# kaushik87599/Melo-GAN

Hardware: AMD Instinct MI355X
Metric: piano-roll samples/sec (G+D step), batch=64 128x256 roll (higher is better)
Workload: dtype f32; 1 GPU; cfg2: 128x256 piano-roll, batch=64 per GPU, full G+D+emotion-D step (1 critic update incl. gradient penalty + 1 generator update); global_batch=64, T=256, C=128, parallelism=dp1, graph=True

## Files before the change

melo-gan_amd/csrc/wgrad_mfma.hip:

```cpp
#include "common.h"
#include <stdlib.h>
#include <type_traits>

namespace {

struct WgradP {
    const float* s[2];
    const float* l[2];
    int nb[2];
    float* part;
    float* out;
    float* bias_out;
    int Ts, Tl, A, Bc;
    int tt_log2, n_ttiles;
    int bps;
    int n_bgroups;
    int nbg0;
    long slab;
    long wslab;
    int bias_from;
    int nseg_bias;
    int vec_ok;
    int lin;
    int gx, gy, gz;
};

constexpr int RT = 64;
constexpr int BA = 32, BB = 32;

typedef unsigned u32x4 __attribute__((ext_vector_type(4)));

#ifdef MG_STAMPS
__device__ long long* mg_wstamp_buf = nullptr;
#define MG_STAMP(k)                                                                                        \
    do {                                                                                                   \
        if (threadIdx.x == 0 && mg_wstamp_buf)                                                             \
            mg_wstamp_buf[((long)(blockIdx.z * gridDim.y + blockIdx.y) * gridDim.x + blockIdx.x) * 8 + (k)] = \
                wall_clock64();                                                                            \
    } while (0)
#else
#define MG_STAMP(k)
#endif

template <int S, int K>
__device__ __forceinline__ void wgrad_body(const WgradP& p, const int bx, const int by, const int bz) {
    constexpr int PAD = (K - 1) / 2;
    constexpr int RMAX = (RT - 1) * S + K;
    constexpr int NS4 = RT * (BA / 4) / 256;
    constexpr int NL4 = (RMAX * (BB / 4) + 255) / 256 + 1;
    extern __shared__ __attribute__((aligned(16))) float smem[];
    const int tid = threadIdx.x, lane = tid & 63, wave = tid >> 6;
    MG_STAMP(0);
    const int TT = 1 << p.tt_log2, TB = RT >> p.tt_log2;
    const int R = (TT - 1) * S + K;
    const int lrows = TB * R;
    float* Ss = smem;
    float* Ls = smem + RT * BA;
    const int a0 = bx * BA, b0 = by * BB;
    const int split = bz;

    f32x16 acc[K];
#pragma unroll
    for (int k = 0; k < K; ++k)
#pragma unroll
        for (int r = 0; r < 16; ++r) acc[k][r] = 0.f;

    const int h = lane >> 5;
    const int g_begin = split * p.bps;
    const int g_end = min(g_begin + p.bps, p.n_bgroups);
    const int n_chunks = (g_end - g_begin) * p.n_ttiles;

    auto compute = [&]() {
#ifdef MG_EXP_NOMMA
        return;
#endif
#pragma unroll
        for (int r2 = 0; r2 < RT / 8; ++r2) {
            const int r = wave * (RT / 4) + 2 * r2 + h;
            const int seg = r >> p.tt_log2, tl = r & (TT - 1);
            const float av = Ss[r * BA + (lane & 31)];
            const float* lrow = Ls + (seg * R + tl * S) * BB + (lane & 31);
#pragma unroll
            for (int k = 0; k < K; ++k)
                acc[k] = __builtin_amdgcn_mfma_f32_32x32x2f32(av, lrow[k * BB], acc[k], 0, 0, 0);
        }
    };

    const bool fast = ((p.A & 3) == 0) && ((p.Bc & 3) == 0) && p.vec_ok && (lrows * (BB / 4) <= 256 * NL4);
    if (fast) {
        float4 sr[NS4], lr[NL4];
        auto load_chunk = [&](int c) {
            const int g = g_begin + c / p.n_ttiles, tt = c - (c / p.n_ttiles) * p.n_ttiles;
            const int seg_id = g < p.nbg0 ? 0 : 1;
            const int bg = seg_id ? g - p.nbg0 : g;
            const int nb = p.nb[seg_id];
            const int bb0 = bg * TB, t0 = tt * TT, tl0 = t0 * S - PAD;
            const __amdgpu_buffer_rsrc_t srs = __builtin_amdgcn_make_buffer_rsrc(
                const_cast<float*>(seg_id ? p.s[1] : p.s[0]), 0, (int)((long)nb * p.Ts * p.A * 4), 0x00020000);
            const __amdgpu_buffer_rsrc_t lrs = __builtin_amdgcn_make_buffer_rsrc(
                const_cast<float*>(seg_id ? p.l[1] : p.l[0]), 0, (int)((long)nb * p.Tl * p.Bc * 4), 0x00020000);
#pragma unroll
            for (int j = 0; j < NS4; ++j) {
                const int idx = tid + 256 * j;
                const int r = idx / (BA / 4), q = idx - r * (BA / 4);
                const int seg = r >> p.tt_log2, tl = r & (TT - 1);
                const int b = bb0 + seg, t = t0 + tl, a = a0 + 4 * q;
                unsigned off = 0x80000000u;
                if (b < nb && t < p.Ts && a < p.A) off = (unsigned)((((long)b * p.Ts + t) * p.A + a) * 4);
                const u32x4 v = __builtin_amdgcn_raw_buffer_load_b128(srs, off, 0, 0);
                sr[j] = make_float4(__uint_as_float(v[0]), __uint_as_float(v[1]), __uint_as_float(v[2]), __uint_as_float(v[3]));
            }
#pragma unroll
            for (int j = 0; j < NL4; ++j) {
                const int idx = tid + 256 * j;
                const int row = idx / (BB / 4), q = idx - row * (BB / 4);
                const int seg = row / R, rr = row - seg * R;
                const int b = bb0 + seg, t = tl0 + rr, cc = b0 + 4 * q;
                unsigned off = 0x80000000u;
                if (row < lrows && b < nb && t >= 0 && t < p.Tl && cc < p.Bc)
                    off = (unsigned)((((long)b * p.Tl + t) * p.Bc + cc) * 4);
                const u32x4 v = __builtin_amdgcn_raw_buffer_load_b128(lrs, off, 0, 0);
                lr[j] = make_float4(__uint_as_float(v[0]), __uint_as_float(v[1]), __uint_as_float(v[2]), __uint_as_float(v[3]));
            }
        };
        auto store_chunk = [&]() {
#pragma unroll
            for (int j = 0; j < NS4; ++j) *reinterpret_cast<float4*>(Ss + 4 * (tid + 256 * j)) = sr[j];
#pragma unroll
            for (int j = 0; j < NL4; ++j) {
                const int idx = tid + 256 * j;
                if (idx < lrows * (BB / 4)) *reinterpret_cast<float4*>(Ls + 4 * idx) = lr[j];
            }
        };
        if (n_chunks > 0) {
            load_chunk(0);
            store_chunk();
            __syncthreads();
            for (int c = 0; c < n_chunks; ++c) {
                const bool more = c + 1 < n_chunks;
#ifndef MG_EXP_NOLOADS
                if (more) load_chunk(c + 1);
#endif
                compute();
                __syncthreads();
                if (more) {
                    store_chunk();
                    __syncthreads();
                }
            }
        }
    } else {
        for (int g = g_begin; g < g_end; ++g) {
            const int seg_id = g < p.nbg0 ? 0 : 1;
            const int bg = seg_id ? g - p.nbg0 : g;
            const float* Sp = p.s[seg_id];
            const float* Lp = p.l[seg_id];
            const int nb = p.nb[seg_id];
            const int bb0 = bg * TB;
            for (int tt = 0; tt < p.n_ttiles; ++tt) {
                const int t0 = tt * TT;
                const int tl0 = t0 * S - PAD;
                __syncthreads();
                for (int idx = tid; idx < RT * BA; idx += 256) {
                    const int r = idx / BA, al = idx - r * BA;
                    const int seg = r >> p.tt_log2, tl = r & (TT - 1);
                    const int b = bb0 + seg, t = t0 + tl, a = a0 + al;
                    float v = 0.f;
                    if (b < nb && t < p.Ts && a < p.A) v = Sp[((long)b * p.Ts + t) * p.A + a];
                    Ss[r * BA + al] = v;
                }
                for (int idx = tid; idx < TB * R * BB; idx += 256) {
                    const int row = idx / BB, cl = idx - row * BB;
                    const int seg = row / R, rr = row - seg * R;
                    const int b = bb0 + seg, t = tl0 + rr, c = b0 + cl;
                    float v = 0.f;
                    if (b < nb && t >= 0 && t < p.Tl && c < p.Bc) v = Lp[((long)b * p.Tl + t) * p.Bc + c];
                    Ls[row * BB + cl] = v;
                }
                __syncthreads();
                compute();
            }
        }
    }

#ifdef MG_EXP_NOEPI
    if (acc[0][0] != 12345.f) return;
#endif
    MG_STAMP(2);
    float* red = smem;
    float* out = p.part ? p.part + (long)split * p.slab : p.out;
    constexpr int KP = K > 3 ? 3 : K;
    const int nb_cols = min(32, p.Bc - b0);
#pragma unroll
    for (int k0 = 0; k0 < K; k0 += KP) {
        const int kn = (K - k0) < KP ? (K - k0) : KP;
        __syncthreads();
#pragma unroll
        for (int k = k0; k < k0 + kn; ++k)
#pragma unroll
            for (int r = 0; r < 16; ++r)
                red[((wave * KP + (k - k0)) * 32 + (r & 3) + 8 * (r >> 2) + 4 * h) * 33 + (lane & 31)] = acc[k][r];
        __syncthreads();
#pragma unroll 4
        for (int idx = tid; idx < 32 * kn * 32; idx += 256) {
            const int ar = idx / (kn * 32), j = idx - ar * (kn * 32);
            const int bc = j / kn, kk = j - bc * kn;
            const int a = a0 + ar;
            const int o = (kk * 32 + ar) * 33 + bc;
            const float v = (red[o] + red[o + KP * 32 * 33]) + (red[o + 2 * KP * 32 * 33] + red[o + 3 * KP * 32 * 33]);
            if (a < p.A && bc < nb_cols) out[((long)a * p.Bc + b0 + bc) * K + k0 + kk] = v;
        }
    }
    MG_STAMP(3);
}

constexpr int W16_SP = 48;
template <int S> struct W16LP { static constexpr int value = S == 2 ? 40 : 48; };

template <int S, int K>
__device__ __forceinline__ bool wgrad16_applies(const WgradP& p) {
    constexpr int RMAX = (RT - 1) * S + K;
    constexpr int NL4 = (RMAX * (BB / 4) + 255) / 256 + 1;
    const int TT = 1 << p.tt_log2, TB = RT >> p.tt_log2, R = (TT - 1) * S + K;
    return ((p.A & 3) == 0) && ((p.Bc & 3) == 0) && p.vec_ok && (TB * R * (BB / 4) <= 256 * NL4) && p.tt_log2 >= 4;
}

template <int S, int K>
__device__ __forceinline__ void wgrad16_body(const WgradP& p, const int bx, const int by, const int bz) {
    constexpr int PAD = (K - 1) / 2;
    constexpr int RMAX = (RT - 1) * S + K;
    constexpr int NS4 = RT * (BA / 4) / 256;
    constexpr int NL4 = (RMAX * (BB / 4) + 255) / 256 + 1;
    constexpr int SP = W16_SP, LP = W16LP<S>::value;
    extern __shared__ __attribute__((aligned(16))) float smem[];
    const int tid = threadIdx.x, lane = tid & 63, wave = tid >> 6;
    const int li = lane & 15, kq = lane >> 4, wa = wave & 1, wb = wave >> 1;
    const int TT = 1 << p.tt_log2, TB = RT >> p.tt_log2;
    const int R = (TT - 1) * S + K;
    const int lrows = TB * R;
    const int a0 = bx * BA, b0 = by * BB;
    const int g_begin = bz * p.bps, g_end = min(g_begin + p.bps, p.n_bgroups);
    const int n_chunks = (g_end - g_begin) * p.n_ttiles;
    float* out = p.part ? p.part + (long)bz * p.slab : p.out;
    MG_STAMP(0);

    f32x4 acc[K];
#pragma unroll
    for (int k = 0; k < K; ++k) acc[k] = f32x4{0.f, 0.f, 0.f, 0.f};

    if (n_chunks > 0) {
        const int buf_floats = RT * SP + lrows * LP;
        const int sink = 2 * buf_floats + 4 * tid;
        constexpr unsigned DEAD = 0xC0000000u;
        int s_lds[NS4];
        unsigned s_base[NS4];
#pragma unroll
        for (int j = 0; j < NS4; ++j) {
            const int idx = tid + 256 * j, r = idx / (BA / 4), q = idx - r * (BA / 4);
            const int seg = r >> p.tt_log2, tl = r & (TT - 1);
            s_lds[j] = r * SP + 4 * q;
            s_base[j] = (unsigned)((((long)seg * p.Ts + tl) * p.A + a0 + 4 * q) * 4);
            if (a0 + 4 * q >= p.A || (TB > 1 && tl >= p.Ts)) s_base[j] = DEAD;
        }
        int l_lds[NL4], l_ldd[NL4];
        unsigned l_base[NL4];
#pragma unroll
        for (int j = 0; j < NL4; ++j) {
            const int idx = tid + 256 * j, row = idx / (BB / 4), q = idx - row * (BB / 4);
            const int seg = (TB == 1) ? 0 : row / R, rr = row - seg * R;
            const bool live = row < lrows;
            l_lds[j] = live ? RT * SP + row * LP + 4 * q : sink;
            l_ldd[j] = live ? buf_floats : 0;
            l_base[j] = (unsigned)(int)((((long)seg * p.Tl + rr - PAD) * p.Bc + b0 + 4 * q) * 4);
            if (!live || b0 + 4 * q >= p.Bc || (TB > 1 && (rr < PAD || rr - PAD >= p.Tl))) l_base[j] = DEAD;
        }
        f32x4 sr[NS4], lr[NL4];
        __amdgpu_buffer_rsrc_t srs, lrs;
        unsigned s_add = 0, l_add = 0;
        int nc = 0, ng = g_begin, ntt = 0;
        auto chunk_desc = [&]() {
            const int seg_id = ng < p.nbg0 ? 0 : 1;
            const int bg = seg_id ? ng - p.nbg0 : ng;
            const int bb0 = bg * TB;
            const int nbv = min(TB, p.nb[seg_id] - bb0);
            srs = __builtin_amdgcn_make_buffer_rsrc(const_cast<float*>((seg_id ? p.s[1] : p.s[0]) + (long)bb0 * p.Ts * p.A), 0,
                                                    nbv * p.Ts * p.A * 4, 0x00020000);
            lrs = __builtin_amdgcn_make_buffer_rsrc(const_cast<float*>((seg_id ? p.l[1] : p.l[0]) + (long)bb0 * p.Tl * p.Bc), 0,
                                                    nbv * p.Tl * p.Bc * 4, 0x00020000);
            const int t0 = ntt << p.tt_log2;
            s_add = (unsigned)(t0 * p.A * 4);
            l_add = (unsigned)(t0 * S * p.Bc * 4);
        };
        auto chunk_next = [&]() {
            if (nc + 1 < n_chunks) {
                ++nc;
                if (++ntt == p.n_ttiles) { ntt = 0; ++ng; }
            }
            chunk_desc();
        };
        auto bload = [&](const __amdgpu_buffer_rsrc_t& rsrc, unsigned off) {
            const u32x4 v = __builtin_amdgcn_raw_buffer_load_b128(rsrc, off, 0, 0);
            return f32x4{__uint_as_float(v[0]), __uint_as_float(v[1]), __uint_as_float(v[2]), __uint_as_float(v[3])};
        };
        auto lds4 = [&](int off) { return reinterpret_cast<f32x4*>(__builtin_assume_aligned(smem + off, 16)); };
        auto store_s = [&](int j, int buf) { *lds4(s_lds[j] + (buf ? buf_floats : 0)) = sr[j]; };
        auto store_l = [&](int j, int buf) { *lds4(l_lds[j] + (buf ? l_ldd[j] : 0)) = lr[j]; };

        const int abase = kq * SP + 16 * wa + li;
        const int lbase = RT * SP + kq * S * LP + 16 * wb + li;
        constexpr int NG = RT / 4;
        constexpr int NOPS = 2 * (NS4 + NL4);
        typedef float f32x8 __attribute__((ext_vector_type(8)));
        f32x8 fr[2];
        auto block_off = [&](int g) { return (((4 * g) >> p.tt_log2) * R + ((4 * g) & (TT - 1)) * S) * LP; };
        auto read_a = [&](int boff, int g, f32x8& v) { v[7] = smem[boff + abase + 4 * g * SP]; };
        auto read_b = [&](int boff, int g, int k, f32x8& v) { v[k] = smem[boff + lbase + block_off(g) + k * LP]; };
        auto chunk = [&](auto parity, int c) {
            constexpr int P = decltype(parity)::value;
            const int cur = P ? buf_floats : 0, oth = buf_floats - cur;
            chunk_next();
#pragma unroll
            for (int m = 0; m < NG * K; ++m) {
                const int g = m / K, k = m % K;
                acc[k] = __builtin_amdgcn_mfma_f32_16x16x4f32(fr[g & 1][7], fr[g & 1][k], acc[k], 0, 0, 0);
                const int gn = g + 1 < NG ? g + 1 : 0, bo = g + 1 < NG ? cur : oth;
                if (g + 1 == NG && k == 0) __syncthreads();
                if (k == 0) read_a(bo, gn, fr[(g + 1) & 1]);
                read_b(bo, gn, k, fr[(g + 1) & 1]);
                if (g + 1 < NG && k == K - 1) {
#pragma unroll
                    for (int o = 0; o < NOPS; ++o) {
                        if (o * (NG - 1) / NOPS != g) continue;
                        const int j = o / 2;
                        if (j < NS4) {
                            if (o % 2 == 0) store_s(j, 1 - P);
                            else sr[j] = bload(srs, s_base[j] + s_add);
                        } else {
                            if (o % 2 == 0) store_l(j - NS4, 1 - P);
                            else lr[j - NS4] = bload(lrs, l_base[j - NS4] + l_add);
                        }
                    }
                }
                __builtin_amdgcn_sched_barrier(0);
            }
        };
        auto load_all = [&]() {
#pragma unroll
            for (int j = 0; j < NS4; ++j) sr[j] = bload(srs, s_base[j] + s_add);
#pragma unroll
            for (int j = 0; j < NL4; ++j) lr[j] = bload(lrs, l_base[j] + l_add);
        };
        chunk_desc();
        load_all();
#pragma unroll
        for (int j = 0; j < NS4; ++j) store_s(j, 0);
#pragma unroll
        for (int j = 0; j < NL4; ++j) store_l(j, 0);
        if (n_chunks > 1) {
            chunk_next();
            load_all();
        }
        __syncthreads();
        read_a(0, 0, fr[0]);
#pragma unroll
        for (int k = 0; k < K; ++k) read_b(0, 0, k, fr[0]);
        MG_STAMP(1);
        for (int c = 0;;) {
            chunk(std::integral_constant<int, 0>{}, c);
            if (++c >= n_chunks) break;
            chunk(std::integral_constant<int, 1>{}, c);
            if (++c >= n_chunks) break;
        }
    }
    MG_STAMP(2);

    __syncthreads();
    constexpr int PE = K * 32 + 1;
    float* red = smem;
#pragma unroll
    for (int k = 0; k < K; ++k)
#pragma unroll
        for (int r = 0; r < 4; ++r) red[(16 * wa + 4 * kq + r) * PE + (16 * wb + li) * K + k] = acc[k][r];
    __syncthreads();
    const int nb_valid = min(32, p.Bc - b0) * K;
#pragma unroll 4
    for (int idx = tid; idx < 32 * K * 32; idx += 256) {
        const int ar = idx / (K * 32), j = idx - ar * (K * 32);
        if (a0 + ar < p.A && j < nb_valid) out[((long)(a0 + ar) * p.Bc + b0) * K + j] = red[ar * PE + j];
    }
    MG_STAMP(3);
}

constexpr int LIN_BB = 128;
__device__ __forceinline__ bool wgrad_lin_applies(const WgradP& p) {
    return p.lin != 0;
}
__device__ __forceinline__ void wgrad_lin_body(const WgradP& p, const int bx, const int by, const int bz) {
    extern __shared__ __attribute__((aligned(16))) float smem[];
    constexpr int SPL = 36, LPL = 132;
    float* Ss = smem;
    float* Ls = smem + RT * SPL;
    const int tid = threadIdx.x, lane = tid & 63, wave = tid >> 6, h = lane >> 5, c = lane & 31;
    const int a0 = bx * BA, b0 = by * LIN_BB;
    const int TB = RT;
    const int g_begin = bz * p.bps, g_end = min(g_begin + p.bps, p.n_bgroups);
    f32x16 acc;
#pragma unroll
    for (int i = 0; i < 16; ++i) acc[i] = 0.f;
    for (int g = g_begin; g < g_end; ++g) {
        const int seg_id = g < p.nbg0 ? 0 : 1;
        const int bb0 = (seg_id ? g - p.nbg0 : g) * TB;
        const int nb = p.nb[seg_id];
        const float* Sp = p.s[seg_id] + (long)bb0 * p.A;
        const float* Lp = p.l[seg_id] + (long)bb0 * p.Bc;
        const int rows = min(TB, nb - bb0);
        __syncthreads();
#pragma unroll
        for (int j = 0; j < 2; ++j) {
            const int idx = tid + 256 * j, r = idx >> 3, q = idx & 7;
            const bool ok = r < rows && a0 + 4 * q < p.A;
            const f32x4 v = *reinterpret_cast<const f32x4*>(Sp + (long)(ok ? r : 0) * p.A + (ok ? a0 + 4 * q : 0));
            *reinterpret_cast<f32x4*>(Ss + r * SPL + 4 * q) = ok ? v : f32x4{0.f, 0.f, 0.f, 0.f};
        }
#pragma unroll
        for (int j = 0; j < 8; ++j) {
            const int idx = tid + 256 * j, r = idx >> 5, q = idx & 31;
            const bool ok = r < rows && b0 + 4 * q < p.Bc;
            const f32x4 v = *reinterpret_cast<const f32x4*>(Lp + (long)(ok ? r : 0) * p.Bc + (ok ? b0 + 4 * q : 0));
            *reinterpret_cast<f32x4*>(Ls + r * LPL + 4 * q) = ok ? v : f32x4{0.f, 0.f, 0.f, 0.f};
        }
        __syncthreads();
#pragma unroll 8
        for (int r2 = 0; r2 < RT / 2; ++r2) {
            const int r = 2 * r2 + h;
            acc = __builtin_amdgcn_mfma_f32_32x32x2f32(Ss[r * SPL + c], Ls[r * LPL + 32 * wave + c], acc, 0, 0, 0);
        }
    }
    float* out = p.part ? p.part + (long)bz * p.slab : p.out;
    const int b = b0 + 32 * wave + c;
    if (b < p.Bc) {
#pragma unroll
        for (int i = 0; i < 16; ++i) {
            const int a = a0 + (i & 3) + 8 * (i >> 2) + 4 * h;
            if (a < p.A) out[(long)a * p.Bc + b] = acc[i];
        }
    }
}

__device__ __forceinline__ void wgrad_bias_body(const WgradP& p, const int cb, const int bz) {
    extern __shared__ __attribute__((aligned(16))) float smem[];
    f32x4* bred = reinterpret_cast<f32x4*>(smem);
    const int tid = threadIdx.x, q = tid & 7, rl = tid >> 3;
    const bool from_s = p.bias_from == 1;
    const int C = from_s ? p.A : p.Bc, T = from_s ? p.Ts : p.Tl;
    const int TB = RT >> p.tt_log2;
    const int g_begin = bz * p.bps, g_end = min(g_begin + p.bps, p.n_bgroups);
    f32x4 acc = {0.f, 0.f, 0.f, 0.f};
    const int c = cb * 32 + 4 * q;
    for (int seg = 0; seg < p.nseg_bias && seg < 2; ++seg) {
        const int gs = seg ? p.nbg0 : 0, ge = seg ? p.n_bgroups : p.nbg0;
        const int ga = max(g_begin, gs), gb = min(g_end, ge);
        if (ga >= gb) continue;
        const int b_lo = (ga - gs) * TB, b_hi = min((gb - gs) * TB, p.nb[seg]);
        const float* base = (from_s ? p.s[seg] : p.l[seg]) + (long)b_lo * T * C;
        const long rows = (long)(b_hi - b_lo) * T;
        if (c + 3 < C && (C & 3) == 0 && p.vec_ok) {
            long r = rl;
            for (; r + 32 * 7 < rows; r += 32 * 8) {
                f32x4 v[8];
#pragma unroll
                for (int u = 0; u < 8; ++u) v[u] = *reinterpret_cast<const f32x4*>(base + (r + 32 * u) * C + c);
#pragma unroll
                for (int u = 0; u < 8; ++u) acc += v[u];
            }
            for (; r < rows; r += 32) acc += *reinterpret_cast<const f32x4*>(base + r * C + c);
        } else {
            for (long r = rl; r < rows; r += 32)
#pragma unroll
                for (int e = 0; e < 4; ++e)
                    if (c + e < C) acc[e] += base[r * C + c + e];
        }
    }
    bred[tid] = acc;
    __syncthreads();
    if (tid < 32) {
        const int ch = cb * 32 + tid;
        if (ch < C) {
            float v = 0.f;
#pragma unroll 8
            for (int g = 0; g < 32; ++g) v += bred[8 * g + (tid >> 2)][tid & 3];
            if (p.part) p.part[(long)bz * p.slab + p.wslab + ch] = v;
            else p.bias_out[ch] = v;
        }
    }
}

struct WgradJobs {
    WgradP p[MG_MAX_WGRAD_JOBS];
    int first[MG_MAX_WGRAD_JOBS + 1];
    int bfirst[MG_MAX_WGRAD_JOBS + 1];
    int n;
};
template <int S, int K>
__global__ __launch_bounds__(256, 2) void wgrad_multi_kernel(const WgradJobs J) {
    const int bid = (int)blockIdx.x;
    const bool tile = bid < J.first[J.n];
    const int* first = tile ? J.first : J.bfirst;
    int j = 0;
    while (j + 1 < J.n && bid >= first[j + 1]) ++j;
    const int b = bid - first[j];
    const WgradP& p = J.p[j];
    if (tile) {
        const int gxy = p.gx * p.gy, bz = b / gxy, r = b - bz * gxy;
        if (K == 1 && wgrad_lin_applies(p)) wgrad_lin_body(p, r % p.gx, r / p.gx, bz);
        else if (wgrad16_applies<S, K>(p)) wgrad16_body<S, K>(p, r % p.gx, r / p.gx, bz);
        else wgrad_body<S, K>(p, r % p.gx, r / p.gx, bz);
    } else {
        const int ncb = ((p.bias_from == 1 ? p.A : p.Bc) + 31) >> 5;
        wgrad_bias_body(p, b % ncb, b / ncb);
    }
}

struct ReduceJobs {
    const float* part[MG_MAX_WGRAD_JOBS];
    float* out[MG_MAX_WGRAD_JOBS];
    float* bias_out[MG_MAX_WGRAD_JOBS];
    long n[MG_MAX_WGRAD_JOBS], wn[MG_MAX_WGRAD_JOBS];
    int nsplit[MG_MAX_WGRAD_JOBS];
    int first[MG_MAX_WGRAD_JOBS + 1];
    int njobs;
};
__global__ __launch_bounds__(256) void reduce_slabs_multi_kernel(const ReduceJobs J) {
    __shared__ float sh[4][64];
    int j = 0;
    while (j + 1 < J.njobs && (int)blockIdx.x >= J.first[j + 1]) ++j;
    const float* __restrict__ part = J.part[j];
    const long n = J.n[j], wn = J.wn[j];
    const int nsplit = J.nsplit[j];
    const int ex = threadIdx.x & 63, g = threadIdx.x >> 6;
    const long i = (long)((int)blockIdx.x - J.first[j]) * 64 + ex;
    float s = 0.f;
    if (i < n)
        for (int z = g; z < nsplit; z += 4) s += part[(long)z * n + i];
    sh[g][ex] = s;
    __syncthreads();
    if (g == 0 && i < n) {
        const float v = (sh[0][ex] + sh[1][ex]) + (sh[2][ex] + sh[3][ex]);
        if (i < wn) J.out[j][i] = v;
        else J.bias_out[j][i - wn] = v;
    }
}

struct Plan {
    int tt_log2, TB, n_ttiles, nbg0, nbg1, nsplit, bps;
};

constexpr int MAX_SPLITS = 32;

Plan make_plan(int A, int Bc, int K, int nb0, int nb1, int Ts, long want_slices = 0) {
    Plan pl;
    int lg = mg_ilog2_ceil(Ts);
    const int lgrt = mg_ilog2_ceil(RT);
    if (lg > lgrt) lg = lgrt;
    pl.tt_log2 = lg;
    pl.TB = RT >> lg;
    pl.n_ttiles = (int)mg_cdiv(Ts, 1 << lg);
    pl.nbg0 = (int)mg_cdiv(nb0, pl.TB);
    pl.nbg1 = nb1 > 0 ? (int)mg_cdiv(nb1, pl.TB) : 0;
    const int ngroups = pl.nbg0 + pl.nbg1;
    const long tiles = mg_cdiv(A, BA) * mg_cdiv(Bc, BB);
    long target = 256;
    if (const char* f = getenv("MG_WGRAD_TARGET")) target = atol(f);
    long want = want_slices > 0 ? want_slices : mg_cdiv(target, tiles);
    long max_by_work = ((long)ngroups * pl.n_ttiles) / 2;
    if (max_by_work < 1) max_by_work = 1;
    if (want > max_by_work) want = max_by_work;
    if (want > ngroups) want = ngroups;
    if (want > MAX_SPLITS) want = MAX_SPLITS;
    if (want < 1) want = 1;
    pl.bps = (int)mg_cdiv(ngroups, want);
    pl.nsplit = (int)mg_cdiv(ngroups, pl.bps);
    return pl;
}

}

#ifdef MG_STAMPS
extern "C" int mg_dbg_set_wstamps(long long* buf) {
    return hipMemcpyToSymbol(HIP_SYMBOL(mg_wstamp_buf), &buf, sizeof(buf)) == hipSuccess ? 0 : 1;
}
#endif

extern "C" size_t mg_wgrad_workspace_bytes(int A, int Bc, int K, int nb_total, int Ts) {
    int lg = mg_ilog2_ceil(Ts);
    const int lgrt = mg_ilog2_ceil(RT);
    if (lg > lgrt) lg = lgrt;
    const int TB = RT >> lg;
    long ns = mg_cdiv(nb_total, TB) + 1;
    if (ns > MAX_SPLITS) ns = MAX_SPLITS;
    return (size_t)ns * ((size_t)A * (size_t)Bc * (size_t)K + (size_t)(A > Bc ? A : Bc)) * sizeof(float);
}

namespace {
int build_wgrad(const float* s0, const float* l0, int nb0, const float* s1, const float* l1, int nb1, float* out,
                float* bias_out, int bias_from, int Ts, int Tl, int A, int Bc, int K, int stride, void* work,
                size_t work_bytes, WgradP& p, Plan& pl, size_t& lds, dim3& grid, long want_slices = 0) {
    MG_CHECK_ARG(bias_from >= 0 && bias_from <= 2 && ((bias_from == 0) == (bias_out == nullptr)),
                 "mg_wgrad: bias_out and bias_from (1: sums of S, 2: sums of L) must be given together");
    MG_CHECK_ARG(s0 && l0 && out && nb0 > 0, "mg_wgrad: null/empty segment 0");
    MG_CHECK_ARG(nb1 == 0 || (s1 && l1), "mg_wgrad: null segment 1");
    MG_CHECK_ARG(Ts > 0 && Tl > 0 && A > 0 && Bc > 0, "mg_wgrad: bad shape");
    MG_CHECK_ARG(K == 1 || K == 3 || K == 5, "mg_wgrad: K=%d unsupported", K);
    MG_CHECK_ARG(stride == 1 || stride == 2, "mg_wgrad: stride=%d unsupported", stride);
    if (stride == 2 && K != 5) {
        mg_set_error("mg_wgrad: stride 2 needs K=5");
        return MG_EUNSUP;
    }
    pl = make_plan(A, Bc, K, nb0, nb1, Ts, want_slices);
    const long wslab = (long)A * Bc * K;
    const long slab = wslab + (bias_from == 1 ? A : bias_from == 2 ? Bc : 0);
    if (pl.nsplit > 1 && (!work || work_bytes < (size_t)pl.nsplit * slab * sizeof(float))) {
        mg_set_error("mg_wgrad: workspace too small (%zu < %zu)", work_bytes, (size_t)pl.nsplit * slab * sizeof(float));
        return MG_EWORK;
    }
    p = WgradP{};
    p.s[0] = s0; p.l[0] = l0; p.nb[0] = nb0;
    p.s[1] = s1; p.l[1] = l1; p.nb[1] = nb1;
    p.part = pl.nsplit > 1 ? (float*)work : nullptr;
    p.out = out;
    p.bias_out = bias_out;
    p.Ts = Ts; p.Tl = Tl; p.A = A; p.Bc = Bc;
    p.tt_log2 = pl.tt_log2; p.n_ttiles = pl.n_ttiles;
    p.bps = pl.bps; p.n_bgroups = pl.nbg0 + pl.nbg1; p.nbg0 = pl.nbg0;
    p.slab = slab;
    p.wslab = wslab;
    p.bias_from = bias_from;
    p.nseg_bias = 1;
    const int TT = 1 << pl.tt_log2;
    const int R = (TT - 1) * stride + K;
    size_t lds_floats = 2 * ((size_t)RT * BA + (size_t)pl.TB * R * BB) + 256 * 4;
    const size_t epi_floats = (size_t)4 * (K > 3 ? 3 : K) * 32 * 33;
    if (lds_floats < epi_floats) lds_floats = epi_floats;
    auto ok = [](const float* q, long elems) { return q == nullptr || (((((uintptr_t)q) & 15) == 0) && elems * 4 < (1L << 31)); };
    p.vec_ok = ok(s0, (long)nb0 * Ts * A) && ok(l0, (long)nb0 * Tl * Bc) && ok(nb1 ? s1 : nullptr, (long)nb1 * Ts * A) &&
               ok(nb1 ? l1 : nullptr, (long)nb1 * Tl * Bc) && (long)Tl * Bc * 4 < (1L << 30) && (long)Ts * A * 4 < (1L << 30);
    {
        const int rmax = (RT - 1) * stride + K, nl4 = (rmax * (BB / 4) + 255) / 256 + 1;
        if ((A & 3) == 0 && (Bc & 3) == 0 && p.vec_ok && pl.TB * R * (BB / 4) <= 256 * nl4 && pl.tt_log2 >= 4) {
            const size_t lp16 = stride == 2 ? 40 : 48;
            lds_floats = 2 * ((size_t)RT * W16_SP + (size_t)pl.TB * R * lp16) + 256 * 4;
            const size_t epi16 = (size_t)32 * (K * 32 + 1);
            if (lds_floats < epi16) lds_floats = epi16;
        }
    }
    lds = lds_floats * sizeof(float);
    p.lin = (K == 1 && stride == 1 && Ts == 1 && Tl == 1 && (A & 3) == 0 && (Bc & 3) == 0 && p.vec_ok &&
             mg_cdiv(A, BA) * mg_cdiv(Bc, LIN_BB) >= 128) ? 1 : 0;
    if (p.lin) {
        const size_t lin_floats = (size_t)RT * (36 + 132);
        if (lds < lin_floats * sizeof(float)) lds = lin_floats * sizeof(float);
    }
    p.gx = (int)mg_cdiv(A, BA); p.gy = (int)mg_cdiv(Bc, p.lin ? LIN_BB : BB); p.gz = pl.nsplit;
    const int nbias = bias_from ? pl.nsplit * (int)mg_cdiv(bias_from == 1 ? A : Bc, 32) : 0;
    grid = dim3((unsigned)(p.gx * p.gy * p.gz + nbias));
    return MG_OK;
}
}

extern "C" int mg_wgrad_multi(const mg_wgrad_job* jobs, int n_jobs, int K, int stride, void* work, size_t work_bytes,
                              mg_stream_t stream);

extern "C" int mg_wgrad(const float* s0, const float* l0, int nb0, const float* s1, const float* l1, int nb1,
                        float* out, float* bias_out, int bias_from, int Ts, int Tl, int A, int Bc, int K, int stride,
                        void* work, size_t work_bytes, mg_stream_t stream) {
    mg_wgrad_job j{};
    j.s0 = s0; j.l0 = l0; j.nb0 = nb0;
    j.s1 = s1; j.l1 = l1; j.nb1 = nb1;
    j.out = out; j.bias_out = bias_out; j.bias_from = bias_from;
    j.Ts = Ts; j.Tl = Tl; j.A = A; j.Bc = Bc;
    return mg_wgrad_multi(&j, 1, K, stride, work, work_bytes, stream);
}

extern "C" int mg_wgrad_multi(const mg_wgrad_job* jobs, int n_jobs, int K, int stride, void* work, size_t work_bytes,
                              mg_stream_t stream) {
    MG_CHECK_ARG(jobs && n_jobs > 0 && n_jobs <= MG_MAX_WGRAD_JOBS, "mg_wgrad_multi: 1..%d jobs", MG_MAX_WGRAD_JOBS);
    WgradJobs J{};
    ReduceJobs Rj{};
    size_t lds_max = 0, used = 0;
    int nblocks = 0, rblocks = 0;
    long want[MG_MAX_WGRAD_JOBS];
    {
        long target = 512;
        if (const char* f = getenv("MG_WGRAD_TARGET")) target = atol(f);
        long tiles[MG_MAX_WGRAD_JOBS], chunks[MG_MAX_WGRAD_JOBS], total = 0;
        for (int i = 0; i < n_jobs; ++i) {
            const mg_wgrad_job& q = jobs[i];
            MG_CHECK_ARG(q.A > 0 && q.Bc > 0 && q.Ts > 0 && q.Tl > 0 && q.nb0 > 0 && q.nb1 >= 0 && q.s0 && q.l0 && q.out,
                         "mg_wgrad_multi: job %d: null/empty segment 0 or bad shape", i);
            const Plan pl = make_plan(q.A, q.Bc, K, q.nb0, q.nb1, q.Ts);
            tiles[i] = mg_cdiv(q.A, BA) * mg_cdiv(q.Bc, BB);
            chunks[i] = (long)(pl.nbg0 + pl.nbg1) * pl.n_ttiles;
            total += tiles[i] * chunks[i];
        }
        long cpw = mg_cdiv(total, target);
        for (int it = 0; it < 64; ++it) {
            long wgs = 0;
            for (int i = 0; i < n_jobs; ++i) {
                const mg_wgrad_job& q = jobs[i];
                want[i] = (chunks[i] + cpw / 2) / cpw;
                if (want[i] < 1) want[i] = 1;
                const Plan pl = make_plan(q.A, q.Bc, K, q.nb0, q.nb1, q.Ts, want[i]);
                wgs += tiles[i] * pl.nsplit;
            }
            if (wgs <= target) break;
            cpw += mg_cdiv(cpw, 16);
        }
    }
    for (int i = 0; i < n_jobs; ++i) {
        const mg_wgrad_job& q = jobs[i];
        Plan pl;
        size_t lds;
        dim3 grid;
        const size_t need = mg_wgrad_workspace_bytes(q.A, q.Bc, K, q.nb0 + q.nb1, q.Ts);
        void* w = used < work_bytes && work ? (char*)work + used : nullptr;
        const int rc = build_wgrad(q.s0, q.l0, q.nb0, q.s1, q.l1, q.nb1, q.out, q.bias_out, q.bias_from, q.Ts, q.Tl, q.A,
                                   q.Bc, K, stride, w, w ? work_bytes - used : 0, J.p[i], pl, lds, grid, want[i]);
        if (rc != MG_OK) return rc;
        if (pl.nsplit > 1) {
            used += (need + 255) & ~(size_t)255;
            const int r = Rj.njobs++;
            Rj.part[r] = J.p[i].part; Rj.out[r] = q.out; Rj.bias_out[r] = q.bias_out;
            Rj.n[r] = J.p[i].slab; Rj.wn[r] = J.p[i].wslab; Rj.nsplit[r] = pl.nsplit;
            Rj.first[r] = rblocks;
            rblocks += (int)mg_cdiv(J.p[i].slab, 64);
        }
        lds_max = lds > lds_max ? lds : lds_max;
        const int ntile = J.p[i].gx * J.p[i].gy * J.p[i].gz;
        J.first[i] = nblocks;
        nblocks += ntile;
        J.bfirst[i] = (int)grid.x - ntile;
    }
    J.first[n_jobs] = nblocks;
    for (int i = 0; i < n_jobs; ++i) {
        const int nb = J.bfirst[i];
        J.bfirst[i] = nblocks;
        nblocks += nb;
    }
    J.bfirst[n_jobs] = nblocks;
    J.n = n_jobs;
    Rj.first[Rj.njobs] = rblocks;
    hipStream_t st = (hipStream_t)stream;
#define MG_WG(S_, K_) hipLaunchKernelGGL((wgrad_multi_kernel<S_, K_>), dim3((unsigned)nblocks), dim3(256), lds_max, st, J)
    if (stride == 1) {
        if (K == 1) MG_WG(1, 1); else if (K == 3) MG_WG(1, 3); else MG_WG(1, 5);
    } else {
        MG_WG(2, 5);
    }
#undef MG_WG
    MG_CHECK_LAUNCH("wgrad_multi_kernel");
    if (Rj.njobs > 0) {
        hipLaunchKernelGGL(reduce_slabs_multi_kernel, dim3((unsigned)rblocks), dim3(256), 0, st, Rj);
        MG_CHECK_LAUNCH("reduce_slabs_multi_kernel");
    }
    return MG_OK;
}
```

Baseline: 79200 samples/s.

## Deepen wgrad16 global-load prefetch to two register sets and pin params in SGPRs

Measured after the change: 61070 samples/s. -22.9%, worse.

```diff
diff --git a/melo-gan_amd/csrc/wgrad_mfma.hip b/melo-gan_amd/csrc/wgrad_mfma.hip
--- a/melo-gan_amd/csrc/wgrad_mfma.hip
+++ b/melo-gan_amd/csrc/wgrad_mfma.hip
@@ -225,6 +225,12 @@
     return ((p.A & 3) == 0) && ((p.Bc & 3) == 0) && p.vec_ok && (TB * R * (BB / 4) <= 256 * NL4) && p.tt_log2 >= 4;
 }
 
+template <typename T>
+__device__ __forceinline__ T mg_pin_sgpr(T v) {
+    asm volatile("" : "+s"(v));
+    return v;
+}
+
 template <int S, int K>
 __device__ __forceinline__ void wgrad16_body(const WgradP& p, const int bx, const int by, const int bz) {
     constexpr int PAD = (K - 1) / 2;
@@ -274,27 +280,34 @@
             l_base[j] = (unsigned)(int)((((long)seg * p.Tl + rr - PAD) * p.Bc + b0 + 4 * q) * 4);
             if (!live || b0 + 4 * q >= p.Bc || (TB > 1 && (rr < PAD || rr - PAD >= p.Tl))) l_base[j] = DEAD;
         }
-        f32x4 sr[NS4], lr[NL4];
+        const float* const sp0 = mg_pin_sgpr(p.s[0]);
+        const float* const sp1 = mg_pin_sgpr(p.s[1]);
+        const float* const lp0 = mg_pin_sgpr(p.l[0]);
+        const float* const lp1 = mg_pin_sgpr(p.l[1]);
+        const int nb0 = mg_pin_sgpr(p.nb[0]), nb1 = mg_pin_sgpr(p.nb[1]);
+        const int nbg0 = mg_pin_sgpr(p.nbg0), n_tt = mg_pin_sgpr(p.n_ttiles), ttl = mg_pin_sgpr(p.tt_log2);
+        const int s_seq = mg_pin_sgpr(p.Ts * p.A), l_seq = mg_pin_sgpr(p.Tl * p.Bc);
+        const int s_tile = mg_pin_sgpr((p.A * 4) << p.tt_log2), l_tile = mg_pin_sgpr((S * p.Bc * 4) << p.tt_log2);
+
+        f32x4 sr[2][NS4], lr[2][NL4];
         __amdgpu_buffer_rsrc_t srs, lrs;
         unsigned s_add = 0, l_add = 0;
         int nc = 0, ng = g_begin, ntt = 0;
         auto chunk_desc = [&]() {
-            const int seg_id = ng < p.nbg0 ? 0 : 1;
-            const int bg = seg_id ? ng - p.nbg0 : ng;
-            const int bb0 = bg * TB;
-            const int nbv = min(TB, p.nb[seg_id] - bb0);
-            srs = __builtin_amdgcn_make_buffer_rsrc(const_cast<float*>((seg_id ? p.s[1] : p.s[0]) + (long)bb0 * p.Ts * p.A), 0,
-                                                    nbv * p.Ts * p.A * 4, 0x00020000);
-            lrs = __builtin_amdgcn_make_buffer_rsrc(const_cast<float*>((seg_id ? p.l[1] : p.l[0]) + (long)bb0 * p.Tl * p.Bc), 0,
-                                                    nbv * p.Tl * p.Bc * 4, 0x00020000);
-            const int t0 = ntt << p.tt_log2;
-            s_add = (unsigned)(t0 * p.A * 4);
-            l_add = (unsigned)(t0 * S * p.Bc * 4);
+            const bool seg1 = ng >= nbg0;
+            const int bb0 = (seg1 ? ng - nbg0 : ng) * TB;
+            int nbv = min(TB, (seg1 ? nb1 : nb0) - bb0);
+            if (nc >= n_chunks) nbv = 0;
+            srs = __builtin_amdgcn_make_buffer_rsrc(const_cast<float*>((seg1 ? sp1 : sp0) + (long)bb0 * s_seq), 0, nbv * s_seq * 4,
+                                                    0x00020000);
+            lrs = __builtin_amdgcn_make_buffer_rsrc(const_cast<float*>((seg1 ? lp1 : lp0) + (long)bb0 * l_seq), 0, nbv * l_seq * 4,
+                                                    0x00020000);
+            s_add = (unsigned)(ntt * s_tile);
+            l_add = (unsigned)(ntt * l_tile);
         };
         auto chunk_next = [&]() {
-            if (nc + 1 < n_chunks) {
-                ++nc;
-                if (++ntt == p.n_ttiles) { ntt = 0; ++ng; }
+            if (++nc < n_chunks) {
+                if (++ntt == n_tt) { ntt = 0; ++ng; }
             }
             chunk_desc();
         };
@@ -303,8 +316,8 @@
             return f32x4{__uint_as_float(v[0]), __uint_as_float(v[1]), __uint_as_float(v[2]), __uint_as_float(v[3])};
         };
         auto lds4 = [&](int off) { return reinterpret_cast<f32x4*>(__builtin_assume_aligned(smem + off, 16)); };
-        auto store_s = [&](int j, int buf) { *lds4(s_lds[j] + (buf ? buf_floats : 0)) = sr[j]; };
-        auto store_l = [&](int j, int buf) { *lds4(l_lds[j] + (buf ? l_ldd[j] : 0)) = lr[j]; };
+        auto store_s = [&](int j, int buf, const f32x4& v) { *lds4(s_lds[j] + (buf ? buf_floats : 0)) = v; };
+        auto store_l = [&](int j, int buf, const f32x4& v) { *lds4(l_lds[j] + (buf ? l_ldd[j] : 0)) = v; };
 
         const int abase = kq * SP + 16 * wa + li;
         const int lbase = RT * SP + kq * S * LP + 16 * wb + li;
@@ -312,10 +325,10 @@
         constexpr int NOPS = 2 * (NS4 + NL4);
         typedef float f32x8 __attribute__((ext_vector_type(8)));
         f32x8 fr[2];
-        auto block_off = [&](int g) { return (((4 * g) >> p.tt_log2) * R + ((4 * g) & (TT - 1)) * S) * LP; };
+        auto block_off = [&](int g) { return (((4 * g) >> ttl) * R + ((4 * g) & (TT - 1)) * S) * LP; };
         auto read_a = [&](int boff, int g, f32x8& v) { v[7] = smem[boff + abase + 4 * g * SP]; };
         auto read_b = [&](int boff, int g, int k, f32x8& v) { v[k] = smem[boff + lbase + block_off(g) + k * LP]; };
-        auto chunk = [&](auto parity, int c) {
+        auto chunk = [&](auto parity) {
             constexpr int P = decltype(parity)::value;
             const int cur = P ? buf_floats : 0, oth = buf_floats - cur;
             chunk_next();
@@ -333,44 +346,44 @@
                         if (o * (NG - 1) / NOPS != g) continue;
                         const int j = o / 2;
                         if (j < NS4) {
-                            if (o % 2 == 0) store_s(j, 1 - P);
-                            else sr[j] = bload(srs, s_base[j] + s_add);
+                            if (o % 2 == 0) store_s(j, 1 - P, sr[P][j]);
+                            else sr[P][j] = bload(srs, s_base[j] + s_add);
                         } else {
-                            if (o % 2 == 0) store_l(j - NS4, 1 - P);
-                            else lr[j - NS4] = bload(lrs, l_base[j - NS4] + l_add);
+                            if (o % 2 == 0) store_l(j - NS4, 1 - P, lr[P][j - NS4]);
+                            else lr[P][j - NS4] = bload(lrs, l_base[j - NS4] + l_add);
                         }
                     }
                 }
                 __builtin_amdgcn_sched_barrier(0);
             }
         };
-        auto load_all = [&]() {
-#pragma unroll
-            for (int j = 0; j < NS4; ++j) sr[j] = bload(srs, s_base[j] + s_add);
-#pragma unroll
-            for (int j = 0; j < NL4; ++j) lr[j] = bload(lrs, l_base[j] + l_add);
+        auto load_all = [&](int set) {
+#pragma unroll
+            for (int j = 0; j < NS4; ++j) sr[set][j] = bload(srs, s_base[j] + s_add);
+#pragma unroll
+            for (int j = 0; j < NL4; ++j) lr[set][j] = bload(lrs, l_base[j] + l_add);
         };
         chunk_desc();
-        load_all();
-#pragma unroll
-        for (int j = 0; j < NS4; ++j) store_s(j, 0);
-#pragma unroll
-        for (int j = 0; j < NL4; ++j) store_l(j, 0);
-        if (n_chunks > 1) {
-            chunk_next();
-            load_all();
-        }
+        load_all(1);
+        chunk_next();
+        load_all(0);
+#pragma unroll
+        for (int j = 0; j < NS4; ++j) store_s(j, 0, sr[1][j]);
+#pragma unroll
+        for (int j = 0; j < NL4; ++j) store_l(j, 0, lr[1][j]);
+        chunk_next();
+        load_all(1);
         __syncthreads();
         read_a(0, 0, fr[0]);
 #pragma unroll
         for (int k = 0; k < K; ++k) read_b(0, 0, k, fr[0]);
         MG_STAMP(1);
-        for (int c = 0;;) {
-            chunk(std::integral_constant<int, 0>{}, c);
-            if (++c >= n_chunks) break;
-            chunk(std::integral_constant<int, 1>{}, c);
-            if (++c >= n_chunks) break;
-        }
+        int c = 0;
+        for (; c + 2 <= n_chunks; c += 2) {
+            chunk(std::integral_constant<int, 0>{});
+            chunk(std::integral_constant<int, 1>{});
+        }
+        if (c < n_chunks) chunk(std::integral_constant<int, 0>{});
     }
     MG_STAMP(2);
 
```
